# ddemidov/vexcl

Hardware: AMD Instinct MI355X
Metric: fp64 CSR SpMV GFLOP/s, 3D Poisson 512^3 (y = A*x through vex::SpMat's library object vexhip_spmat) (higher is better)
Workload: dtype f64

## Files before the change

### vexcl_amd/csrc/common.hpp

```cpp
#pragma once
#include <hip/hip_runtime.h>
#include <algorithm>
#include <chrono>
#include <cstdint>
#include <cstdio>
#include <cstdlib>
#include <string>

#include "../../include/vexhip.h"

namespace vexhip {

std::string &last_error();
int &last_error_code();
int fail(const char *file, int line, const std::string &what);

inline int check(hipError_t e, const char *file, int line) {
    if (e == hipSuccess) return 0;
    (void)hipGetLastError();
    const int rc = fail(file, line, std::string(hipGetErrorName(e)) + ": " + hipGetErrorString(e));
    last_error_code() = (int)e;
    return rc;
}

constexpr int kWave = 64;

inline hipStream_t as_stream(void *s) { return reinterpret_cast<hipStream_t>(s); }

struct device_info {
    int cus = 0;
    bool ok = false;
};
const device_info &info(int dev);


enum env_id {
    ENV_VEXCL_CACHE_DIR,
    ENV_VEXCL_CACHE_KERNELS,
    ENV_VEXCL_SHOW_KERNELS,
    ENV_VEXCL_SHOW_SCRATCH,
    ENV_VEXHIP_COMM_PEER,
    ENV_VEXHIP_DEBUG,
    ENV_VEXHIP_DIST_PACK,
    ENV_VEXHIP_FFT_EXTRA_LDS,
    ENV_VEXHIP_FFT_LANES_DIV,
    ENV_VEXHIP_FFT_NO_SINGLE,
    ENV_VEXHIP_FFT_ROW_ELEMS,
    ENV_VEXHIP_FFT_STRIDED_ELEMS,
    ENV_VEXHIP_GRID32_DEPTH,
    ENV_VEXHIP_GRID_2D_LINE,
    ENV_VEXHIP_GRID_BUILD_WGS,
    ENV_VEXHIP_GRID_SEGMENT,
    ENV_VEXHIP_HALO_ACQUIRE,
    ENV_VEXHIP_HALO_DEBUG,
    ENV_VEXHIP_HALO_DEPTH,
    ENV_VEXHIP_HALO_EDGE_PLANES,
    ENV_VEXHIP_HALO_HI_PLANES,
    ENV_VEXHIP_HALO_LO_PLANES,
    ENV_VEXHIP_HALO_NO_GHOST,
    ENV_VEXHIP_HALO_NO_PUSH,
    ENV_VEXHIP_HALO_PUSH_BLOCKS,
    ENV_VEXHIP_HALO_TWO_LAUNCHES,
    ENV_VEXHIP_HALO_TWO_PASS,
    ENV_VEXHIP_IPC_PUSH_PER_BLOCK,
    ENV_VEXHIP_IPC_TIMEOUT_MS,
    ENV_VEXHIP_IPC_WINDOW_MEM,
    ENV_VEXHIP_MALLOC_STAGGER,
    ENV_VEXHIP_MARCH_LDS,
    ENV_VEXHIP_MARCH_RUN,
    ENV_VEXHIP_NO_GRID,
    ENV_VEXHIP_NO_GRID_BUILD,
    ENV_VEXHIP_NO_PLANE512,
    ENV_VEXHIP_PLANE32_DEPTH,
    ENV_VEXHIP_PLANE_DEPTH,
    ENV_VEXHIP_PLANE_FORCE,
    ENV_VEXHIP_PLANE_STORE,
    ENV_VEXHIP_PLANE_TILE,
    ENV_VEXHIP_RCCL_SELF,
    ENV_VEXHIP_SELL_XLOAD,
    ENV_VEXHIP_SETUP_TRACE,
    ENV_COUNT
};
const char *env(env_id id);
void reload_env();

struct setup_trace {
    bool on; hipStream_t s; std::chrono::steady_clock::time_point t0, last;
    explicit setup_trace(hipStream_t st) : on(env(ENV_VEXHIP_SETUP_TRACE) != nullptr), s(st) { t0 = last = std::chrono::steady_clock::now(); }
    void mark(const char *what) {
        if (!on) return;
        (void)hipStreamSynchronize(s);
        const auto now = std::chrono::steady_clock::now();
        std::fprintf(stderr, "[vexhip set-up] %-28s %8.3f ms  (at %8.3f)\n", what,
                     std::chrono::duration<double, std::milli>(now - last).count(), std::chrono::duration<double, std::milli>(now - t0).count());
        last = now;
    }
};

template <typename T> struct dev_buf {
    T *p = nullptr;
    dev_buf() = default;
    dev_buf(const dev_buf &) = delete;
    dev_buf &operator=(const dev_buf &) = delete;
    ~dev_buf() { if (p) (void)hipFree(p); }
    hipError_t alloc(size_t count) { return hipMalloc(reinterpret_cast<void **>(&p), std::max<size_t>(count, 1) * sizeof(T)); }
    hipError_t free_now() { T *q = p; p = nullptr; return q ? hipFree(q) : hipSuccess; }
    T *release() { T *r = p; p = nullptr; return r; }
};

int scan_exclusive_i32_internal(int dev, hipStream_t s, const int *in, int *out, int64_t n);
int scan_exclusive_u32_tmp(hipStream_t s, const unsigned *in, unsigned *out, int64_t n, unsigned *tmp);
size_t scan_tmp_elems_u32(int64_t n);

}

#define VEXHIP_TRY(expr)                                                      \
    do {                                                                      \
        if (int _rc = ::vexhip::check((expr), __FILE__, __LINE__)) return _rc;\
    } while (0)

#define VEXHIP_REQUIRE(cond, msg)                                             \
    do {                                                                      \
        if (!(cond)) return ::vexhip::fail(__FILE__, __LINE__, msg);          \
    } while (0)

#define VEXHIP_SET_DEVICE(dev) VEXHIP_TRY(hipSetDevice(dev))

#define VEXHIP_WARM_TU(name)                                                   \
    namespace vexhip {                                                         \
    namespace { __global__ void warm_##name##_kernel() {} }                    \
    void warm_##name() { warm_##name##_kernel<<<1, 64>>>(); }                  \
    }

#define VEXHIP_LAUNCH_CHECK() VEXHIP_TRY(hipGetLastError())
```

### vexcl_amd/csrc/plane.hip

```cpp
#include "common.hpp"
#include "walk.hpp"
#include "halo.hpp"
#include "plane.hpp"
#include "storage.hpp"

#include <algorithm>
#include <cstdlib>
#include <cstring>
#include <vector>

namespace vexhip {
namespace {

constexpr int PL_LINE_B = PL_ROWS * 8;

__device__ __forceinline__ void push_piece(const double *__restrict__ x, int far, const halo_dev &H, unsigned long long step, bool down, int j,
        int per, unsigned target, bool counted, int *s_flag)
{
    const int t = threadIdx.x;
    if (t == 0) *s_flag = spin_until(down ? H.sent_lo : H.sent_hi, step - 1ull, H.err, H.ticks, 0) ? 1 : 0;
    __syncthreads();
    if (!*s_flag) return;
    const double *src = x + (down ? (long long)H.z0 * far : (long long)(H.z1 - 1) * far);
    double *dst = down ? H.dst_lo : H.dst_hi;
    const int i0 = j * per, i1 = i0 + per < H.halo ? i0 + per : H.halo;
    for (int i = i0 + 2 * t; i < i1; i += 512)
        *reinterpret_cast<d2 *>(dst + i) = *reinterpret_cast<const d2 *>(src + i);
    __builtin_amdgcn_fence(__ATOMIC_RELEASE, "workgroup");
    asm volatile("s_waitcnt vmcnt(0)" ::: "memory");
    __syncthreads();
    if (t == 0 && counted) {
        unsigned *cnt = H.done + (down ? 1 : 2);
        const unsigned old = __hip_atomic_fetch_add(cnt, 1u, __ATOMIC_RELAXED, __HIP_MEMORY_SCOPE_AGENT);
        if (old + 1u == target) {
            __hip_atomic_store(cnt, 0u, __ATOMIC_RELAXED, __HIP_MEMORY_SCOPE_AGENT);
            if (H.release) __builtin_amdgcn_fence(__ATOMIC_RELEASE, "");
            __hip_atomic_store(down ? H.peer_arrive_lo : H.peer_arrive_hi, step, __ATOMIC_RELAXED, __HIP_MEMORY_SCOPE_SYSTEM);
        }
    }
}

template <int TY, int ZM, int STORE_AUX, bool HALO, bool FLAT = false>
__device__ __forceinline__
void plane_walk(const double *__restrict__ x, double *__restrict__ y, double alpha, const double *__restrict__ zs, double beta,
        const int *__restrict__ blocks, const char *__restrict__ pool, const int *__restrict__ deltas, const double *__restrict__ values,
        const plane_dev &pd, const halo_dev &H, [[maybe_unused]] const unsigned long long step_in)
{
    __shared__ int s_slot[256];
    __shared__ double s_value[256];
    __shared__ double s_other[15][256];

    const int t = threadIdx.x;
    unsigned b = blockIdx.x;
    [[maybe_unused]] unsigned long long step = 0;
    [[maybe_unused]] __shared__ int s_flag[2];
    [[maybe_unused]] unsigned long long dbg_t0 = 0, dbg_flag = 0, dbg_data = 0;
    if constexpr (HALO) {
        if (H.debug) dbg_t0 = wall_clock64();
        step = step_in;
        halo_announce(H, step);
        const unsigned npush = H.pull ? 0u : (H.dst_lo ? (unsigned)H.push_blocks : 0u) + (H.dst_hi ? (unsigned)H.push_blocks : 0u);
        if (b < npush) {
            const bool down = H.dst_lo && b < (unsigned)H.push_blocks;
            const unsigned j = down ? b : b - (H.dst_lo ? (unsigned)H.push_blocks : 0u);
            const int per = ((H.halo + H.push_blocks - 1) / H.push_blocks + 511) / 512 * 512;
            push_piece(x, pd.far, H, step, down, (int)j, per, (unsigned)H.push_blocks, true, &s_flag[0]);
            if (H.debug && t == 0) { unsigned long long *d = H.debug + 6ull * blockIdx.x; d[0] = dbg_t0; d[1] = 0; d[2] = 0; d[3] = wall_clock64(); d[4] = ~0ull; d[5] = down ? 0ull : 1ull; }
            return;
        }
        b -= npush;
    }
    const unsigned xcd = b & 7u, q = b >> 3;
    const int zc = (int)(q / (unsigned)pd.tpx), tyl = (int)(q - (unsigned)zc * (unsigned)pd.tpx);
    const int tile = (int)xcd * pd.tpx + tyl;
    if (tile >= pd.tiles) return;
    const int y0 = TY * tile;
    int z, zend;
    [[maybe_unused]] bool second = false;
    [[maybe_unused]] int z2 = 0, zend2 = 0;
    if constexpr (HALO) {
        const int mid0 = H.z0 + H.lo_planes, mid1 = H.z1 - H.hi_planes;
        const int nmain = (mid1 - mid0 + pd.depth - 1) / pd.depth;
        if (zc < nmain) { z = mid0 + zc * pd.depth; zend = z + pd.depth < mid1 ? z + pd.depth : mid1; }
        else if (H.hi_planes && zc == nmain) { z = mid1; zend = H.z1; }
        else if (H.lo_two_pass && mid0 - H.z0 >= 2) {
            z = H.z0 + 1; zend = mid0; second = true; z2 = H.z0; zend2 = H.z0 + 1;
        } else { z = H.z0; zend = mid0; }
    } else {
        z = zc * pd.depth;
        zend = z + pd.depth < pd.nz ? z + pd.depth : pd.nz;
    }
    if (z >= zend) return;
    [[maybe_unused]] const int z_first0 = z, mid_end = zend;
    if constexpr (HALO) {
        if (!H.pull && H.push_blocks == 0 && b < 512u) {
            const bool down = b < 256u;
            double *dst = down ? H.dst_lo : H.dst_hi;
            if (dst) {
                const int per = ((H.halo + 255) / 256 + 511) / 512 * 512, j = (int)(b & 255u);
                push_piece(x, pd.far, H, step, down, j, per, (unsigned)((H.halo + per - 1) / per), j * per < H.halo, &s_flag[0]);
                __syncthreads();
            }
        }
    }
    const int ny = pd.ny;
    const int nslices = (int)pd.nslices, xlines = (int)pd.xlines;
    const long long x_last = pd.x_last;
    const unsigned lane_b = 16u * (unsigned)t;
    const int edge_b = (t >> 6) * 1024 + ((t & 63) == 63 ? 1024 : -8);

    s_slot[t] = 2 * position_of(deltas[t], pd.far); s_value[t] = values[t];
    __syncthreads();

    const int wp = (pd.w + 1) >> 1;
    auto decode = [&](int blk) -> unsigned {
        if (pd.pitch > 0) return decode_table<false>(pool + (long long)blk * 7 * pd.pitch + 2 * t, pd.pitch, s_value, s_other, t);
        const unsigned *cw = reinterpret_cast<const unsigned *>(pool + (long long)blk * ((long long)wp * 2048)) + t;
        unsigned dcw[4], vcw[4];
#pragma unroll
        for (int u = 0; u < 4; ++u) { dcw[u] = u < wp ? cw[u * 256] : 0xffffffffu; vcw[u] = u < wp ? cw[(wp + u) * 256] : 0u; }
#pragma unroll
        for (int p = 0; p < 14; ++p) s_other[p][t] = 0.0;
        unsigned bits = 0;
#pragma unroll
        for (int j = 0; j < 8; ++j) {
            const unsigned cword = dcw[j >> 1] >> (16 * (j & 1)), vword = vcw[j >> 1] >> (16 * (j & 1));
#pragma unroll
            for (int r = 0; r < 2; ++r) {
                const unsigned code = j < pd.w ? (cword >> (8 * r)) & 255u : 255u;
                const bool real = code < PL_PAD_FIRST;
                const int slot = real ? s_slot[code] + r : 14;
                s_other[slot][t] = s_value[real ? (vword >> (8 * r)) & 255u : 255u];
                bits |= (real ? 1u : 0u) << slot;
            }
        }
        return bits & 0x3fffu;
    };

    const int hot = pd.hot;
    double aH[7][2];
    unsigned long long mH[7][2];
    take_hot(decode(hot), s_other, t, aH, mH);
    unsigned bitsO = 0;
    int other = -1;

    const int line_lo = HALO ? H.z0 * ny : 0, line_hi = HALO ? H.z1 * ny : xlines;
    const int yline_hi = HALO ? H.z1 * ny : nslices;
    [[maybe_unused]] bool got_lo = false, got_hi = false, ghost_bad = false;
    auto line_of = [&](int zz, int l) -> int {
        int li = zz * ny + (y0 - 1 + l);
        li = li < line_lo ? line_lo : li; li = li >= line_hi ? line_hi - 1 : li;
        return li;
    };
    auto ld = [&](int zz, int l) -> d2 {
        if constexpr (HALO) {
            const int li = zz * ny + (y0 - 1 + l);
            if (li < line_lo || li >= line_hi) {
                const bool below = li < line_lo;
                const int gl = below ? li - (line_lo - ny) : li - line_hi;
                const double *g = below ? H.lo : H.hi;
                d2 r = {0.0, 0.0};
                if (!g || gl < 0 || gl >= ny || l == 0 || l == TY + 1) return r;
                bool &got = below ? got_lo : got_hi;
                if (!got && H.pull != 2) {
                    if (t == 0) s_flag[below ? 0 : 1] = spin_until(below ? H.arrive_lo : H.arrive_hi, step, H.err, H.ticks, H.acquire) ? 1 : 0;
                    __syncthreads();
                    if (!s_flag[below ? 0 : 1]) ghost_bad = true;
                    got = true;
                    if (H.debug && !dbg_flag) dbg_flag = wall_clock64();
                }
                if (ghost_bad) { r.x = r.y = __builtin_nan(""); return r; }
                if (H.debug && !dbg_data) {
                    const d2 v = *reinterpret_cast<const d2 *>(reinterpret_cast<const char *>(g + (long long)gl * PL_ROWS) + lane_b);
                    asm volatile("s_waitcnt vmcnt(0)" :: "v"(v.x), "v"(v.y) : "memory");
                    dbg_data = wall_clock64();
                    return v;
                }
                return *reinterpret_cast<const d2 *>(reinterpret_cast<const char *>(g + (long long)gl * PL_ROWS) + lane_b);
            }
        }
        const char *p = reinterpret_cast<const char *>(x + (long long)line_of(zz, l) * PL_ROWS);
        return *reinterpret_cast<const d2 *>(p + lane_b);
    };
    auto edge = [&](int zz, int l) -> double {
        if constexpr (HALO) {
            const int li = zz * ny + (y0 - 1 + l);
            if (li < line_lo || li >= line_hi) return 0.0;
            long long i = (long long)li * PL_ROWS + (edge_b >> 3);
            const long long a = (long long)line_lo * PL_ROWS, e = (long long)line_hi * PL_ROWS - 1;
            i = i < a ? a : i; i = i > e ? e : i;
            return x[i];
        }
        long long i = (long long)line_of(zz, l) * PL_ROWS + (edge_b >> 3);
        i = i < 0 ? 0 : i; i = i > x_last ? x_last : i;
        return x[i];
    };
    auto yold = [&](int zz, int l) -> d2 {
        int li = zz * ny + (y0 + l);
        li = li < line_lo ? line_lo : li; li = li >= yline_hi ? yline_hi - 1 : li;
        return *reinterpret_cast<const d2 *>(reinterpret_cast<const char *>(zs + (long long)li * PL_ROWS) + lane_b);
    };

    constexpr int NPASS = HALO ? 2 : 1;
    for (int pass = 0; pass < NPASS; ++pass) {
    if constexpr (HALO) if (pass == 1) { if (!second) break; z = z2; zend = zend2; }
    d2 Cs[4][TY], Hs[2][2], Yo[TY];
    double Es[2][TY];
    const unsigned plane_b32 = (unsigned)ny * (unsigned)PL_LINE_B;
    const int z_first = z;
    const __amdgpu_buffer_rsrc_t rx = __builtin_amdgcn_make_buffer_rsrc(
        const_cast<double *>(x + ((long long)z_first * ny + (y0 - 1)) * PL_ROWS), 0, -1, 0x00020000);
    const __amdgpu_buffer_rsrc_t ry = __builtin_amdgcn_make_buffer_rsrc(y + ((long long)z_first * ny + y0) * PL_ROWS, 0, -1, 0x00020000);
    [[maybe_unused]] const __amdgpu_buffer_rsrc_t rz = __builtin_amdgcn_make_buffer_rsrc(const_cast<double *>(ZM == 1 ? zs : x) + ((long long)z_first * ny + y0) * PL_ROWS, 0, -1, 0x00020000);
    fill_registers<ZM>(Cs, Hs, Es, Yo, z, !FLAT, ld, edge, yold);

    int zh = zend;
    {
        const int a = (line_hi - 1 - TY - y0) / ny - 3, bb = (yline_hi - TY - y0) / ny - (ZM == 1 ? 1 : 0);
        if (line_hi - 1 - TY - y0 < 0 || yline_hi - TY - y0 < 0) zh = 0;
        else { zh = zh < a + 1 ? zh : a + 1; zh = zh < bb + 1 ? zh : bb + 1; }
    }

    while (z < zend) {
        unsigned long long use_hot[TY];
        const int run = fast_run(blocks, ny, y0, TY, z, zh, hot, other, t, use_hot);
        if (run >= 4) {
            unsigned xo = (unsigned)((z + 2 - z_first) * plane_b32), yo = (unsigned)((z - z_first) * plane_b32);
            auto fast_step = [&](d2 (&P)[TY], d2 (&C)[TY], d2 (&N)[TY], d2 (&Hl)[2], double (&E)[TY]) {
                d2 o[TY];
#pragma unroll
                for (int l = 0; l < TY; ++l) {
                    double xs[2][7], s[2] = {};
                    stencil_x(P, C, N, Hl, E, l, xs);
                    if (use_hot[l] & 1ull) hot_sums(s, aH, mH, xs); else other_sums(s, s_other, t, bitsO, xs);
                    o[l] = add_addend<ZM>(alpha, s, beta, Yo[l], C[l]);
                }
#pragma unroll
                for (int l = 0; l < TY; ++l) use_hot[l] >>= 1;
#pragma unroll
                for (int l = 0; l < TY; ++l) store16<STORE_AUX>(o[l], ry, (int)lane_b, yo + l * PL_LINE_B);
                if (ZM == 1) {
#pragma unroll
                    for (int l = 0; l < TY; ++l) Yo[l] = load16<double>(rz, (int)lane_b, yo + plane_b32 + l * PL_LINE_B);
                }
                if constexpr (!FLAT) {
                    Hl[0] = load16<double>(rx, (int)lane_b, xo);
                    Hl[1] = load16<double>(rx, (int)lane_b, xo + (TY + 1) * PL_LINE_B);
                }
#pragma unroll
                for (int l = 0; l < TY; ++l) {
                    P[l] = load16<double>(rx, (int)lane_b, xo + plane_b32 + (l + 1) * PL_LINE_B);
                    E[l] = load_edge<double>(rx, edge_b + 8, xo + (l + 1) * PL_LINE_B - 8u);
                }
                xo += plane_b32; yo += plane_b32; ++z;
            };
            for (int g = run >> 2; g > 0; --g) fast_group(fast_step, Cs, Hs, Es);
            if (run == 64) continue;
        }
        if (z >= zend) break;
#pragma unroll
        for (int l = 0; l < TY; ++l) {
            const int li = z * ny + (y0 + l);
            if (li < yline_hi) {
                double xs[2][7], s[2] = {};
                stencil_x(Cs[0], Cs[1], Cs[2], Hs[0], Es[0], l, xs);
                const int blk = __builtin_amdgcn_readfirstlane(blocks[li]);
                if (blk == hot) hot_sums(s, aH, mH, xs);
                else {
                    if (blk != other) { bitsO = decode(blk); other = blk; }
                    other_sums(s, s_other, t, bitsO, xs);
                }
                const d2 o = add_addend<ZM>(alpha, s, beta, Yo[l], Cs[1][l]);
                __builtin_nontemporal_store(o, reinterpret_cast<d2 *>(reinterpret_cast<char *>(y + (long long)li * PL_ROWS) + lane_b));
            }
        }
        rotate_by_copy<ZM>(Cs, Hs, Es, Yo, z, !FLAT, ld, edge, yold);
        ++z;
    }
    }
    if constexpr (HALO) {
        if (H.debug && t == 0) {
            unsigned long long *d = H.debug + 6ull * blockIdx.x;
            d[0] = dbg_t0; d[1] = dbg_flag; d[2] = dbg_data; d[3] = wall_clock64(); d[4] = (unsigned long long)(second ? z2 : z_first0); d[5] = (unsigned long long)(second ? mid_end : zend);
        }
    }
}

#ifndef VEXHIP_HALO_WAVES
#define VEXHIP_HALO_WAVES 2
#endif
template <int TY, int ZM, int STORE_AUX, bool HALO = false, bool FLAT = false>
__global__ __launch_bounds__(256, (TY == 2 && !HALO) ? 4 : (HALO ? VEXHIP_HALO_WAVES : 2))
void sell8_plane_kernel(const double *__restrict__ x, double *__restrict__ y, double alpha, const double *__restrict__ zs, double beta,
        const int *__restrict__ blocks, const char *__restrict__ pool, const int *__restrict__ deltas, const double *__restrict__ values,
        plane_dev pd, halo_dev H)
{
    if constexpr (!HALO) {
        plane_walk<TY, ZM, STORE_AUX, false, FLAT>(x, y, alpha, zs, beta, blocks, pool, deltas, values, pd, H, 0ull);
    } else {
        const unsigned long long step = *H.step;
        plane_walk<TY, ZM, STORE_AUX, true>(x, y, alpha, zs, beta, blocks, pool, deltas, values, pd, H, step);
        halo_finish(H, step);
    }
}

__global__ __launch_bounds__(256)
void stream_copy_kernel(const double *__restrict__ x, double *__restrict__ y, long long npairs, long long n) {
    const long long i = (long long)blockIdx.x * 256 + threadIdx.x;
    if (i < npairs) __builtin_nontemporal_store(reinterpret_cast<const d2 *>(x)[i], reinterpret_cast<d2 *>(y) + i);
    else if (i == npairs && (n & 1)) y[n - 1] = x[n - 1];
}

__global__ void halo_signal_kernel(halo_dev H) {
    const unsigned long long step = *H.step;
    if (H.consumed_lo) __hip_atomic_store(H.consumed_lo, step, __ATOMIC_RELEASE, __HIP_MEMORY_SCOPE_SYSTEM);
    if (H.consumed_hi) __hip_atomic_store(H.consumed_hi, step, __ATOMIC_RELEASE, __HIP_MEMORY_SCOPE_SYSTEM);
    if (H.pull == 1) {
        if (H.sent_lo) (void)spin_until(H.sent_lo, step, H.err, H.ticks, 0);
        if (H.sent_hi) (void)spin_until(H.sent_hi, step, H.err, H.ticks, 0);
    }
    *H.step = step + 1ull;
}

}
}

namespace vexhip {
int plane_apply_axpby(int dev, void *stream, int64_t n, double alpha, int zm, const double *zs, double beta, int64_t w, const void *pool,
        const int32_t *blocks, const int32_t *deltas, const double *values, const double *x, double *y, const vexhip_plane *plane)
{
    if (int rc = plane_check(plane, 0, PL_LINE_B, n, w, pool && blocks && deltas && values, x, y, true)) return rc;
    VEXHIP_REQUIRE(zm == 0 || zm == 2 || (zm == 1 && zs && (reinterpret_cast<uintptr_t>(zs) & 15) == 0), "plane product: the addend must be a 16-byte aligned vector");
    VEXHIP_SET_DEVICE(dev);
    const plane_dev pd = plane_launch(*plane, n, w, plane->tile, plane->depth);
    unsigned grid;
    if (int rc = plane_workgroups(pd, pd.nz, 0, 0, &grid)) return rc;
    const char *cpool = static_cast<const char *>(pool);
    with_launch_forms(zm, plane->store_policy, [&](auto ZM, auto AUX) {
        auto kernel = plane->tile == 4 ? sell8_plane_kernel<4, ZM(), AUX()> : plane->flat ? sell8_plane_kernel<2, ZM(), AUX(), false, true> : sell8_plane_kernel<2, ZM(), AUX()>;
        kernel<<<grid, 256, 0, as_stream(stream)>>>(x, y, alpha, zs, beta, blocks, cpool, deltas, values, pd, halo_dev());
    });
    VEXHIP_LAUNCH_CHECK();
    return 0;
}

}

using namespace vexhip;

static bool plane_geometry_with(long long cus, long long ny, long long nz, int hot, vexhip_plane *out);
static bool plane_geometry(int dev, long long ny, long long nz, int hot, vexhip_plane *out)
{
    return plane_geometry_with(std::max(1, info(dev).cus), ny, nz, hot, out);
}
static bool plane_geometry_with(long long cus, long long ny, long long nz, int hot, vexhip_plane *out)
{
    cus = std::max(1ll, cus);
    auto depth_for = [&](long long tl) {
        const long long tiles = ny / tl;
        long long chunks = std::max(1ll, std::min(nz / 8, (cus + tiles / 2) / tiles));
        if (tiles * chunks > cus || tiles * chunks * 20 < cus * 19) {
            double best = 0;
            const long long cmax = std::max(1ll, nz / 16);
            for (long long c = 1; c <= cmax; ++c) {
                const long long per_cu = (tiles * c + cus - 1) / cus;
                if (per_cu < 6 && c < cmax) continue;
                const double est = (double)per_cu * (double)((nz + c - 1) / c + 6);
                if (best == 0 || est <= best * 1.01) { if (best == 0 || est < best) best = est; chunks = c; }
                if (per_cu > 24) break;
            }
        }
        if (chunks == 1 && nz >= 32 && nz <= 192 && tiles * 2 <= 2 * cus) chunks = 2;
        return (nz + chunks - 1) / chunks;
    };
    long long tile = 2;
    if (const char *e = env(ENV_VEXHIP_PLANE_TILE)) tile = (std::atoi(e) == 4 && ny % 4 == 0) ? 4 : 2;
    long long depth = depth_for(tile);
    if (const char *e = env(ENV_VEXHIP_PLANE_DEPTH)) depth = std::max(1, std::atoi(e));
    depth = std::min(depth, nz);
    while ((depth + 4) * ny * PL_LINE_B >= (1ll << 32) && depth > 8) depth = (depth + 1) / 2;
    if ((depth + 4) * ny * PL_LINE_B >= (1ll << 32)) return false;
    out->lines_per_plane = (int32_t)ny; out->planes = (int32_t)nz; out->depth = (int32_t)depth; out->hot_block = hot; out->tile = (int32_t)tile;
    out->store_policy = tile == 4 ? 2 : 1;
    if (const char *e = env(ENV_VEXHIP_PLANE_STORE)) out->store_policy = std::max(0, std::min(3, std::atoi(e)));
    return true;
}

namespace vexhip {
int plane_plan_from_grid(int dev, const vexhip_grid *grid, int64_t rows, vexhip_plane *out)
{
    VEXHIP_REQUIRE(grid && out, "NULL argument");
    std::memset(out, 0, sizeof(*out));
    const bool force = env(ENV_VEXHIP_PLANE_FORCE) != nullptr;
    if (!grid->usable || grid->nx != PL_ROWS || grid->segments != 1 || rows % PL_ROWS != 0) return 0;
    const long long ny = grid->lines_per_plane, nz = grid->planes;
    if (ny < 4 || ny % 2 != 0 || (nz < 4 && !force) || (rows / PL_ROWS < 64 && !force)) return 0;
    if ((grid->x_last + 1) % PL_ROWS != 0 || grid->x_last + 1 < rows) return 0;
    if (!plane_geometry(dev, ny, nz, grid->hot_class, out)) return 0;
    out->table_pitch = grid->pitch;
    out->flat = grid->flat;
    out->x_last = grid->x_last; out->usable = 1;
    return 0;
}
}

namespace vexhip {
int plane_apply_halo(int dev, hipStream_t s, int64_t n_ext, double alpha, int append, int64_t w, const void *pool, const int32_t *blocks,
        const int32_t *deltas, const double *values, const double *x, double *y, const vexhip_plane *plane, halo_dev H)
{
    if (int rc = plane_check(plane, 2, PL_LINE_B, n_ext, w, pool && blocks && deltas && values, x, y, true)) return rc;
    if (int rc = check_halo_step(H, plane->planes, (long long)plane->lines_per_plane * PL_ROWS, false)) return rc;
    VEXHIP_SET_DEVICE(dev);
    const int nzr = H.z1 - H.z0;
    int edge_planes = 8;
    if (const char *e = env(ENV_VEXHIP_HALO_EDGE_PLANES)) edge_planes = std::max(1, std::atoi(e));
    int lo_planes = edge_planes, hi_planes = edge_planes;
    if (const char *e = env(ENV_VEXHIP_HALO_LO_PLANES)) lo_planes = std::max(1, std::atoi(e));
    if (const char *e = env(ENV_VEXHIP_HALO_HI_PLANES)) hi_planes = std::max(1, std::atoi(e));
    H.lo_planes = H.lo ? std::min(lo_planes, nzr) : 0;
    H.hi_planes = H.hi ? std::min(hi_planes, nzr - H.lo_planes) : 0;
    const int mid = nzr - H.lo_planes - H.hi_planes;
    int depth = std::max(1, mid);
    if (const char *e = env(ENV_VEXHIP_HALO_DEPTH)) depth = std::max(1, std::atoi(e));
    const plane_dev pd = plane_launch(*plane, n_ext, w, 2, depth);
    const long long npush = H.pull ? 0 : (H.dst_lo ? H.push_blocks : 0) + (H.dst_hi ? H.push_blocks : 0);
    unsigned grid;
    if (int rc = plane_workgroups(pd, mid, (H.lo_planes ? 1 : 0) + (H.hi_planes ? 1 : 0), npush, &grid)) return rc;
    VEXHIP_REQUIRE(H.pull || H.push_blocks > 0 || grid - npush >= 512 || !(H.dst_lo || H.dst_hi), "too few workgroups to push the boundary planes");
    const double *xe = x - (long long)H.z0 * pd.far;
    double *ye = y - (long long)H.z0 * pd.far;
    const char *cpool = static_cast<const char *>(pool);
    auto kernel = append ? sell8_plane_kernel<2, 1, 18, true> : sell8_plane_kernel<2, 0, 18, true>;
    kernel<<<grid, 256, 0, s>>>(xe, ye, alpha, append ? ye : nullptr, append ? 1.0 : 0.0, blocks, cpool, deltas, values, pd, H);
    VEXHIP_LAUNCH_CHECK();
    if (H.pull != 2 && !H.one_launch) {
        halo_signal_kernel<<<1, 1, 0, s>>>(H);
        VEXHIP_LAUNCH_CHECK();
    }
    return 0;
}
}

extern "C" {

int vexhip_sell8_plane_geometry(int cus, int64_t lines_per_plane, int64_t planes, vexhip_plane *out)
{
    VEXHIP_REQUIRE(out, "NULL output");
    std::memset(out, 0, sizeof(*out));
    reload_env();
    VEXHIP_REQUIRE(lines_per_plane >= 4 && lines_per_plane % 2 == 0 && lines_per_plane < (1ll << 30) && planes >= 1 && planes < (1ll << 30), "bad grid");
    if (!plane_geometry_with(cus, lines_per_plane, planes, 0, out)) { std::memset(out, 0, sizeof(*out)); return 0; }
    return 0;
}

int vexhip_sell8_plane_plan(int dev, void *stream, const int32_t *deltas, int ndeltas, const int32_t *blocks, int64_t nslices,
        const void *pool, int64_t dictionary_blocks, int64_t ell_width, int64_t rows, int64_t tail_nnz, int value_bytes,
        int64_t x_last, vexhip_plane *out)
{
    VEXHIP_REQUIRE(out, "NULL output");
    std::memset(out, 0, sizeof(*out));
    reload_env();
    const bool force = env(ENV_VEXHIP_PLANE_FORCE) != nullptr;
    if ((value_bytes != 8 && value_bytes != 4) || !deltas || !blocks || !pool || ndeltas < 2 || ndeltas > 7 || dictionary_blocks < 1 || dictionary_blocks > 128) return 0;
    if (ell_width < 1 || ell_width > 8 || tail_nnz != 0 || rows != nslices * PL_ROWS || (nslices < 64 && !force)) return 0;
    if (x_last < 0 || (x_last + 1) % PL_ROWS != 0 || x_last + 1 < rows) return 0;
    VEXHIP_SET_DEVICE(dev);
    hipStream_t s = as_stream(stream);
    const int wp = (int)((ell_width + 1) / 2);
    const size_t code_bytes = (size_t)wp * 2048;
    std::vector<int> table((size_t)ndeltas), id((size_t)nslices);
    std::vector<unsigned> codes((size_t)dictionary_blocks * code_bytes / 4);
    VEXHIP_TRY(hipMemcpyAsync(table.data(), deltas, sizeof(int) * (size_t)ndeltas, hipMemcpyDeviceToHost, s));
    VEXHIP_TRY(hipMemcpyAsync(id.data(), blocks, sizeof(int) * (size_t)nslices, hipMemcpyDeviceToHost, s));
    VEXHIP_TRY(hipMemcpyAsync(codes.data(), pool, (size_t)dictionary_blocks * code_bytes, hipMemcpyDeviceToHost, s));
    VEXHIP_TRY(hipStreamSynchronize(s));
    long long far = 0;
    for (int d : table) {
        const long long a = std::llabs((long long)d);
        if (a == 0 || a == 1 || a == PL_ROWS) continue;
        if (far == 0) far = a;
        if (a != far) return 0;
    }
    if (far < 4 * PL_ROWS || far % (2 * PL_ROWS) != 0 || far > (1ll << 30)) return 0;
    const long long ny = far / PL_ROWS, nz = (nslices + ny - 1) / ny;
    if (nz < 4 && !force) return 0;
    auto position = [&](int d) { return d == 0 ? 3 : d == -1 ? 2 : d == 1 ? 4 : d == -PL_ROWS ? 1 : d == PL_ROWS ? 5 : d == -far ? 0 : 6; };
    for (int64_t blk = 0; blk < dictionary_blocks; ++blk) {
        const unsigned *cw = codes.data() + (size_t)blk * code_bytes / 4;
        for (int t = 0; t < 256; ++t)
            for (int r = 0; r < 2; ++r) {
                int last = -1;
                for (int j = 0; j < (int)ell_width; ++j) {
                    const unsigned cword = cw[(size_t)(j >> 1) * 256 + t] >> (16 * (j & 1));
                    const unsigned code = (cword >> (8 * r)) & 255u;
                    if (code >= PL_PAD_FIRST) continue;
                    if ((int)code >= ndeltas) return 0;
                    const int p = position(table[code]);
                    if (p <= last) return 0;
                    last = p;
                }
            }
    }
    std::vector<int64_t> uses((size_t)dictionary_blocks, 0);
    for (int64_t k = 0; k < nslices; ++k) {
        if (id[(size_t)k] < 0 || id[(size_t)k] >= dictionary_blocks) return 0;
        ++uses[(size_t)id[(size_t)k]];
    }
    const int hot = (int)(std::max_element(uses.begin(), uses.end()) - uses.begin());
    if ((nslices - uses[(size_t)hot]) * 16 > nslices && !force) return 0;
    if (!plane_geometry(dev, ny, nz, hot, out)) return 0;
    out->flat = 1;
    for (int d : table) if (std::llabs((long long)d) == PL_ROWS) out->flat = 0;
    out->x_last = x_last; out->usable = 1;
    return 0;
}

int vexhip_spmv_sell8v_plane_f64_i32(int dev, void *stream, int64_t n, double alpha, int append, int64_t w, const void *pool,
        const int32_t *blocks, const int32_t *deltas, const double *values, const double *x, double *y, const vexhip_plane *plane)
{ return plane_apply<double>(dev, stream, n, alpha, append, w, pool, blocks, deltas, values, x, y, plane); }

int vexhip_stream_copy_f64(int dev, void *stream, const double *x, double *y, int64_t n)
{
    VEXHIP_REQUIRE(n >= 0 && (n == 0 || (x && y)), "bad copy arguments");
    VEXHIP_REQUIRE((reinterpret_cast<uintptr_t>(x) & 15) == 0 && (reinterpret_cast<uintptr_t>(y) & 15) == 0, "stream copy: x and y must be 16-byte aligned");
    if (n == 0) return 0;
    VEXHIP_SET_DEVICE(dev);
    const long long npairs = n / 2, grid = (npairs + 1 + 255) / 256;
    VEXHIP_REQUIRE(grid < (1ll << 31), "vector too large for one launch");
    stream_copy_kernel<<<(unsigned)grid, 256, 0, as_stream(stream)>>>(x, y, npairs, (long long)n);
    VEXHIP_LAUNCH_CHECK();
    return 0;
}

}

VEXHIP_WARM_TU(plane)
```

### vexcl_amd/csrc/runtime.hip

```cpp
#include "common.hpp"

#include <hip/hiprtc.h>

#include <atomic>
#include <cerrno>
#include <cstdlib>
#include <cstring>
#include <fstream>
#include <mutex>
#include <sstream>
#include <unordered_map>
#include <vector>
#include <sys/stat.h>
#include <unistd.h>

namespace vexhip {

std::string &last_error() {
    static thread_local std::string s;
    return s;
}

int &last_error_code() {
    static thread_local int c = 0;
    return c;
}

int fail(const char *file, int line, const std::string &what) {
    std::ostringstream o;
    o << file << ":" << line << "\n\t" << what;
    last_error() = o.str();
    last_error_code() = 0;
    return 1;
}

void warm_misc();
void warm_reduce();
void warm_scan();
void warm_sort();
void warm_stencil();
void warm_ccsr();
void warm_sell8();
void warm_plane();
void warm_plane32();
void warm_grid();
void warm_grid32();
void warm_spmm();
void warm_spmv();
void warm_split();
void warm_comm();
void warm_fft();
void warm_mba();

const device_info &info(int dev) {
    static std::mutex mx;
    static device_info cache[64];
    static device_info fallback;
    std::lock_guard<std::mutex> lock(mx);
    if (dev < 0 || dev >= 64) { fallback.cus = 256; return fallback; }
    if (!cache[dev].ok) {
        hipDeviceProp_t p;
        if (hipGetDeviceProperties(&p, dev) == hipSuccess) {
            cache[dev].cus = p.multiProcessorCount;
            cache[dev].ok = true;
            hipStreamCaptureMode cmode = hipStreamCaptureModeRelaxed;
            const bool swapped = hipThreadExchangeStreamCaptureMode(&cmode) == hipSuccess;
            int cur = -1;
            if (hipGetDevice(&cur) == hipSuccess && hipSetDevice(dev) == hipSuccess) {
                void *d = nullptr;
                if (hipMalloc(&d, 1 << 16) == hipSuccess) {
                    std::vector<char> h(1 << 16);
                    (void)hipMemcpy(h.data(), d, h.size(), hipMemcpyDeviceToHost);
                    (void)hipMemcpy(d, h.data(), h.size(), hipMemcpyHostToDevice);
                    (void)hipFree(d);
                }
                warm_misc(); warm_reduce(); warm_scan(); warm_sort(); warm_stencil(); warm_ccsr(); warm_sell8(); warm_plane(); warm_plane32(); warm_grid(); warm_grid32(); warm_spmm(); warm_spmv(); warm_split(); warm_comm(); warm_fft(); warm_mba();
                (void)hipDeviceSynchronize();
                (void)hipGetLastError();
                (void)hipSetDevice(cur);
            }
            if (swapped) (void)hipThreadExchangeStreamCaptureMode(&cmode);
        } else {
            cache[dev].cus = 256;
        }
    }
    return cache[dev];
}

}

using namespace vexhip;

namespace {

std::atomic<uint64_t> g_compiled{0}, g_disk_hits{0};

std::string digest(const std::string &s) {
    uint64_t h1 = 0xcbf29ce484222325ull, h2 = 0x84222325cbf29ce4ull;
    for (unsigned char c : s) {
        h1 = (h1 ^ c) * 0x100000001b3ull;
        h2 = (h2 ^ (c + 0x9e)) * 0x100000001b3ull;
        h2 ^= h2 >> 29;
    }
    char buf[40];
    std::snprintf(buf, sizeof(buf), "%016llx%016llx", (unsigned long long)h1, (unsigned long long)h2);
    return buf;
}

std::string cache_root() {
    if (const char *e = env(ENV_VEXCL_CACHE_DIR)) return e;
    const char *home = std::getenv("HOME");
    return std::string(home ? home : "/tmp") + "/.vexcl_amd";
}

bool cache_enabled() {
    const char *e = env(ENV_VEXCL_CACHE_KERNELS);
    return !(e && e[0] == '0');
}

bool mkdirs(const std::string &path) {
    std::string cur;
    for (size_t i = 0; i < path.size(); ++i) {
        cur += path[i];
        if (path[i] == '/' || i + 1 == path.size())
            if (::mkdir(cur.c_str(), 0755) != 0 && errno != EEXIST) return false;
    }
    return true;
}

bool read_file(const std::string &p, std::vector<char> &out) {
    std::ifstream f(p, std::ios::binary);
    if (!f) return false;
    f.seekg(0, std::ios::end);
    std::streamsize n = f.tellg();
    if (n <= 0) return false;
    f.seekg(0);
    out.resize((size_t)n);
    return (bool)f.read(out.data(), n);
}

void write_file_atomic(const std::string &dir, const std::string &name, const std::vector<char> &data) {
    if (!mkdirs(dir)) return;
    std::string tmp = dir + "/." + name + "." + std::to_string((long)::getpid());
    {
        std::ofstream f(tmp, std::ios::binary);
        if (!f) return;
        f.write(data.data(), (std::streamsize)data.size());
        if (!f) { ::unlink(tmp.c_str()); return; }
    }
    if (::rename(tmp.c_str(), (dir + "/" + name).c_str()) != 0) ::unlink(tmp.c_str());
}

int rtc_fail(const char *file, int line, hiprtcResult r, const std::string &log) {
    return fail(file, line, std::string("hiprtc: ") + hiprtcGetErrorString(r) + (log.empty() ? "" : "\n" + log));
}

}

namespace vexhip {
namespace {
const char *const kEnvNames[ENV_COUNT] = {
    "VEXCL_CACHE_DIR",
    "VEXCL_CACHE_KERNELS",
    "VEXCL_SHOW_KERNELS",
    "VEXCL_SHOW_SCRATCH",
    "VEXHIP_COMM_PEER",
    "VEXHIP_DEBUG",
    "VEXHIP_DIST_PACK",
    "VEXHIP_FFT_EXTRA_LDS",
    "VEXHIP_FFT_LANES_DIV",
    "VEXHIP_FFT_NO_SINGLE",
    "VEXHIP_FFT_ROW_ELEMS",
    "VEXHIP_FFT_STRIDED_ELEMS",
    "VEXHIP_GRID32_DEPTH",
    "VEXHIP_GRID_2D_LINE",
    "VEXHIP_GRID_BUILD_WGS",
    "VEXHIP_GRID_SEGMENT",
    "VEXHIP_HALO_ACQUIRE",
    "VEXHIP_HALO_DEBUG",
    "VEXHIP_HALO_DEPTH",
    "VEXHIP_HALO_EDGE_PLANES",
    "VEXHIP_HALO_HI_PLANES",
    "VEXHIP_HALO_LO_PLANES",
    "VEXHIP_HALO_NO_GHOST",
    "VEXHIP_HALO_NO_PUSH",
    "VEXHIP_HALO_PUSH_BLOCKS",
    "VEXHIP_HALO_TWO_LAUNCHES",
    "VEXHIP_HALO_TWO_PASS",
    "VEXHIP_IPC_PUSH_PER_BLOCK",
    "VEXHIP_IPC_TIMEOUT_MS",
    "VEXHIP_IPC_WINDOW_MEM",
    "VEXHIP_MALLOC_STAGGER",
    "VEXHIP_MARCH_LDS",
    "VEXHIP_MARCH_RUN",
    "VEXHIP_NO_GRID",
    "VEXHIP_NO_GRID_BUILD",
    "VEXHIP_NO_PLANE512",
    "VEXHIP_PLANE32_DEPTH",
    "VEXHIP_PLANE_DEPTH",
    "VEXHIP_PLANE_FORCE",
    "VEXHIP_PLANE_STORE",
    "VEXHIP_PLANE_TILE",
    "VEXHIP_RCCL_SELF",
    "VEXHIP_SELL_XLOAD",
    "VEXHIP_SETUP_TRACE",
};
struct env_snapshot { bool set[ENV_COUNT]; char text[ENV_COUNT][96]; };
env_snapshot g_env;
std::mutex g_env_mx;
std::once_flag g_env_once;
void read_env() {
    std::lock_guard<std::mutex> lock(g_env_mx);
    for (int i = 0; i < ENV_COUNT; ++i) {
        const char *v = std::getenv(kEnvNames[i]);
        const bool set = v != nullptr;
        if (set == g_env.set[i] && (!set || std::strncmp(g_env.text[i], v, sizeof(g_env.text[i]) - 1) == 0)) continue;
        if (set) { std::strncpy(g_env.text[i], v, sizeof(g_env.text[i]) - 1); g_env.text[i][sizeof(g_env.text[i]) - 1] = 0; }
        g_env.set[i] = set;
    }
}
}
const char *env(env_id id) {
    std::call_once(g_env_once, read_env);
    return g_env.set[id] ? g_env.text[id] : nullptr;
}
void reload_env() {
    std::call_once(g_env_once, read_env);
    read_env();
}
}


extern "C" {

const char *vexhip_last_error(void) { return last_error().c_str(); }
int vexhip_last_error_code(void) { return last_error_code(); }
int vexhip_abi_version(void) { return VEXHIP_ABI_VERSION; }

int vexhip_device_count(int *count) {
    VEXHIP_REQUIRE(count, "count is NULL");
    hipError_t e = hipGetDeviceCount(count);
    if (e == hipErrorNoDevice) { *count = 0; (void)hipGetLastError(); return 0; }
    VEXHIP_TRY(e);
    return 0;
}

int vexhip_device_get_props(int dev, vexhip_device_props *out) {
    VEXHIP_REQUIRE(out, "props is NULL");
    hipDeviceProp_t p;
    VEXHIP_TRY(hipGetDeviceProperties(&p, dev));
    std::memset(out, 0, sizeof(*out));
    std::strncpy(out->name, p.name, sizeof(out->name) - 1);
    std::strncpy(out->arch, p.gcnArchName, sizeof(out->arch) - 1);
    out->compute_units = p.multiProcessorCount;
    out->wavefront_size = p.warpSize;
    out->max_threads_per_block = p.maxThreadsPerBlock;
    out->lds_bytes_per_block = (int32_t)p.sharedMemPerBlock;
    out->clock_khz = p.clockRate;
    out->l2_bytes = p.l2CacheSize;
    out->global_mem_bytes = p.totalGlobalMem;
    out->pci_bus_id = p.pciBusID;
    return 0;
}

int vexhip_device_sync(int dev) {
    VEXHIP_SET_DEVICE(dev);
    VEXHIP_TRY(hipDeviceSynchronize());
    return 0;
}

int vexhip_mem_info(int dev, uint64_t *free_bytes, uint64_t *total_bytes) {
    VEXHIP_SET_DEVICE(dev);
    size_t f = 0, t = 0;
    VEXHIP_TRY(hipMemGetInfo(&f, &t));
    if (free_bytes) *free_bytes = f;
    if (total_bytes) *total_bytes = t;
    return 0;
}

int vexhip_stream_create(int dev, void **stream) {
    VEXHIP_REQUIRE(stream, "stream is NULL");
    VEXHIP_SET_DEVICE(dev);
    hipStream_t s;
    VEXHIP_TRY(hipStreamCreateWithFlags(&s, hipStreamNonBlocking));
    *stream = s;
    return 0;
}

int vexhip_stream_destroy(int dev, void *stream) {
    VEXHIP_SET_DEVICE(dev);
    VEXHIP_TRY(hipStreamDestroy(as_stream(stream)));
    return 0;
}

int vexhip_stream_sync(int dev, void *stream) {
    VEXHIP_SET_DEVICE(dev);
    VEXHIP_TRY(hipStreamSynchronize(as_stream(stream)));
    return 0;
}

int vexhip_event_create(int dev, int timing, void **event) {
    VEXHIP_REQUIRE(event, "event is NULL");
    VEXHIP_SET_DEVICE(dev);
    hipEvent_t e;
    VEXHIP_TRY(hipEventCreateWithFlags(&e, timing ? hipEventDefault : hipEventDisableTiming));
    *event = e;
    return 0;
}

int vexhip_event_destroy(int dev, void *event) {
    VEXHIP_SET_DEVICE(dev);
    VEXHIP_TRY(hipEventDestroy((hipEvent_t)event));
    return 0;
}

int vexhip_event_record(int dev, void *event, void *stream) {
    VEXHIP_SET_DEVICE(dev);
    VEXHIP_TRY(hipEventRecord((hipEvent_t)event, as_stream(stream)));
    return 0;
}

int vexhip_event_sync(int dev, void *event) {
    VEXHIP_SET_DEVICE(dev);
    VEXHIP_TRY(hipEventSynchronize((hipEvent_t)event));
    return 0;
}

int vexhip_stream_wait_event(int dev, void *stream, void *event) {
    VEXHIP_SET_DEVICE(dev);
    VEXHIP_TRY(hipStreamWaitEvent(as_stream(stream), (hipEvent_t)event, 0));
    return 0;
}

int vexhip_event_elapsed_ms(int dev, void *start, void *stop, float *ms) {
    VEXHIP_SET_DEVICE(dev);
    VEXHIP_TRY(hipEventElapsedTime(ms, (hipEvent_t)start, (hipEvent_t)stop));
    return 0;
}


static constexpr size_t kStaggerAlign = size_t(64) << 20, kStaggerStep = size_t(2) << 20, kStaggerSlots = 5, kStaggerFrom = size_t(64) << 20;

extern "C" size_t vexhip_malloc_stagger(size_t bytes, unsigned ordinal) {
    if (bytes < kStaggerFrom) return 0;
    static const bool off = env(ENV_VEXHIP_MALLOC_STAGGER) && std::atoi(env(ENV_VEXHIP_MALLOC_STAGGER)) == 0;
    if (off) return 0;
    return (ordinal % kStaggerSlots) * kStaggerStep;
}
extern "C" size_t vexhip_malloc_placement(size_t bytes, uint64_t raw_address, unsigned ordinal) {
    if (bytes < kStaggerFrom) return 0;
    const uint64_t aligned = (raw_address + kStaggerAlign - 1) / kStaggerAlign * kStaggerAlign;
    return (size_t)(aligned - raw_address) + vexhip_malloc_stagger(bytes, ordinal);
}

namespace {
std::mutex g_alloc_mx;
std::unordered_map<void *, void *> g_alloc_base;
std::atomic<unsigned> g_alloc_ordinal{0};
}

int vexhip_reload_env(void) { reload_env(); return 0; }

int vexhip_malloc(int dev, size_t bytes, void **ptr) {
    VEXHIP_REQUIRE(ptr, "ptr is NULL");
    VEXHIP_SET_DEVICE(dev);
    *ptr = nullptr;
    if (bytes == 0) return 0;
    static const bool off = env(ENV_VEXHIP_MALLOC_STAGGER) && std::atoi(env(ENV_VEXHIP_MALLOC_STAGGER)) == 0;
    if (bytes < kStaggerFrom || off) { VEXHIP_TRY(hipMalloc(ptr, bytes)); return 0; }
    void *raw = nullptr;
    VEXHIP_TRY(hipMalloc(&raw, bytes + kStaggerAlign + (kStaggerSlots - 1) * kStaggerStep));
    const size_t shift = vexhip_malloc_placement(bytes, (uint64_t)reinterpret_cast<uintptr_t>(raw), g_alloc_ordinal.fetch_add(1));
    void *p = static_cast<char *>(raw) + shift;
    if (p != raw) { std::lock_guard<std::mutex> lock(g_alloc_mx); g_alloc_base[p] = raw; }
    *ptr = p;
    return 0;
}

int vexhip_malloc_managed(int dev, size_t bytes, void **ptr) {
    VEXHIP_REQUIRE(ptr, "ptr is NULL");
    VEXHIP_SET_DEVICE(dev);
    *ptr = nullptr;
    if (bytes == 0) return 0;
    VEXHIP_TRY(hipMallocManaged(ptr, bytes, hipMemAttachGlobal));
    return 0;
}

int vexhip_free(int dev, void *ptr) {
    if (!ptr) return 0;
    VEXHIP_SET_DEVICE(dev);
    {
        std::lock_guard<std::mutex> lock(g_alloc_mx);
        auto it = g_alloc_base.find(ptr);
        if (it != g_alloc_base.end()) { ptr = it->second; g_alloc_base.erase(it); }
    }
    VEXHIP_TRY(hipFree(ptr));
    return 0;
}

int vexhip_memcpy_h2d(int dev, void *dst, const void *src, size_t bytes, void *stream, int blocking) {
    if (!bytes) return 0;
    VEXHIP_SET_DEVICE(dev);
    VEXHIP_TRY(hipMemcpyAsync(dst, src, bytes, hipMemcpyHostToDevice, as_stream(stream)));
    if (blocking) VEXHIP_TRY(hipStreamSynchronize(as_stream(stream)));
    return 0;
}

int vexhip_memcpy_d2h(int dev, void *dst, const void *src, size_t bytes, void *stream, int blocking) {
    if (!bytes) return 0;
    VEXHIP_SET_DEVICE(dev);
    VEXHIP_TRY(hipMemcpyAsync(dst, src, bytes, hipMemcpyDeviceToHost, as_stream(stream)));
    if (blocking) VEXHIP_TRY(hipStreamSynchronize(as_stream(stream)));
    return 0;
}

int vexhip_memcpy_d2d(int dev, void *dst, const void *src, size_t bytes, void *stream) {
    if (!bytes) return 0;
    VEXHIP_SET_DEVICE(dev);
    VEXHIP_TRY(hipMemcpyAsync(dst, src, bytes, hipMemcpyDeviceToDevice, as_stream(stream)));
    return 0;
}

int vexhip_memcpy_peer(int dst_dev, void *dst, int src_dev, const void *src, size_t bytes, void *stream) {
    if (!bytes) return 0;
    VEXHIP_SET_DEVICE(dst_dev);
    if (dst_dev == src_dev)
        VEXHIP_TRY(hipMemcpyAsync(dst, src, bytes, hipMemcpyDeviceToDevice, as_stream(stream)));
    else
        VEXHIP_TRY(hipMemcpyPeerAsync(dst, dst_dev, src, src_dev, bytes, as_stream(stream)));
    return 0;
}

int vexhip_memset(int dev, void *ptr, int byte, size_t bytes, void *stream) {
    if (!bytes) return 0;
    VEXHIP_SET_DEVICE(dev);
    VEXHIP_TRY(hipMemsetAsync(ptr, byte, bytes, as_stream(stream)));
    return 0;
}

int vexhip_host_alloc(size_t bytes, void **ptr) {
    VEXHIP_REQUIRE(ptr, "ptr is NULL");
    VEXHIP_TRY(hipHostMalloc(ptr, bytes ? bytes : 1, hipHostMallocDefault));
    return 0;
}

int vexhip_host_free(void *ptr) {
    if (!ptr) return 0;
    VEXHIP_TRY(hipHostFree(ptr));
    return 0;
}


int vexhip_module_compile(int dev, const char *source, const char *options, void **module) {
    reload_env();
    VEXHIP_REQUIRE(source && module, "source/module is NULL");
    VEXHIP_SET_DEVICE(dev);
    hipDeviceProp_t prop;
    VEXHIP_TRY(hipGetDeviceProperties(&prop, dev));
    std::string arch = prop.gcnArchName;
    std::string opts = options ? options : "";

    if (const char *show = env(ENV_VEXCL_SHOW_KERNELS))
        if (show[0] != '0') std::printf("%s\n", source);

    int rtc_major = 0, rtc_minor = 0;
    hiprtcVersion(&rtc_major, &rtc_minor);
    std::string key = digest(std::string(source) + "\x01" + opts + "\x01" + arch + "\x01" +
                             std::to_string(rtc_major) + "." + std::to_string(rtc_minor));
    std::string dir = cache_root() + "/" + key.substr(0, 2) + "/" + key.substr(2);

    std::vector<char> code;
    bool from_disk = cache_enabled() && read_file(dir + "/kernel.hsaco", code);

    if (!from_disk) {
        hiprtcProgram prog;
        hiprtcResult r = hiprtcCreateProgram(&prog, source, "vexcl_kernel.hip", 0, nullptr, nullptr);
        if (r != HIPRTC_SUCCESS) return rtc_fail(__FILE__, __LINE__, r, "");

        std::vector<std::string> ostr;
        ostr.push_back("--offload-arch=" + arch);
        ostr.push_back("-O3");
        ostr.push_back("-std=c++17");
        {
            std::istringstream is(opts);
            std::string tok;
            while (is >> tok) ostr.push_back(tok);
        }
        std::vector<const char *> oc;
        for (auto &s : ostr) oc.push_back(s.c_str());

        r = hiprtcCompileProgram(prog, (int)oc.size(), oc.data());
        if (r != HIPRTC_SUCCESS) {
            size_t ls = 0;
            hiprtcGetProgramLogSize(prog, &ls);
            std::string log(ls, '\0');
            if (ls) hiprtcGetProgramLog(prog, &log[0]);
            hiprtcDestroyProgram(&prog);
            std::fprintf(stderr, "%s\n%s\n", source, log.c_str());
            return rtc_fail(__FILE__, __LINE__, r, log);
        }
        size_t cs = 0;
        r = hiprtcGetCodeSize(prog, &cs);
        if (r != HIPRTC_SUCCESS) { hiprtcDestroyProgram(&prog); return rtc_fail(__FILE__, __LINE__, r, ""); }
        code.resize(cs);
        r = hiprtcGetCode(prog, code.data());
// ... 99 lines not shown
```

Baseline: 4716.

## Add look-ahead plane walk kernel with four-deep block-class prefetch for TY=2

```diff
diff --git a/vexcl_amd/csrc/common.hpp b/vexcl_amd/csrc/common.hpp
--- a/vexcl_amd/csrc/common.hpp
+++ b/vexcl_amd/csrc/common.hpp
@@ -76,6 +76,7 @@
     ENV_VEXHIP_PLANE_FORCE,
     ENV_VEXHIP_PLANE_STORE,
     ENV_VEXHIP_PLANE_TILE,
+    ENV_VEXHIP_PLANE_WALK,
     ENV_VEXHIP_RCCL_SELF,
     ENV_VEXHIP_SELL_XLOAD,
     ENV_VEXHIP_SETUP_TRACE,
diff --git a/vexcl_amd/csrc/plane.hip b/vexcl_amd/csrc/plane.hip
--- a/vexcl_amd/csrc/plane.hip
+++ b/vexcl_amd/csrc/plane.hip
@@ -304,6 +304,204 @@
     }
 }
 
+template <int ZM, int STORE_AUX>
+__device__ __forceinline__
+void plane_walk_ahead(const double *__restrict__ x, double *__restrict__ y, double alpha, const double *__restrict__ zs, double beta,
+        const int *__restrict__ blocks, const char *__restrict__ pool, const int *__restrict__ deltas, const double *__restrict__ values,
+        const plane_dev &pd)
+{
+    constexpr int TY = 2;
+    __shared__ int s_slot[256];
+    __shared__ double s_value[256];
+    __shared__ double s_other[15][256];
+
+    const int t = threadIdx.x;
+    const unsigned b = blockIdx.x;
+    const unsigned xcd = b & 7u, q = b >> 3;
+    const int zc = (int)(q / (unsigned)pd.tpx), tyl = (int)(q - (unsigned)zc * (unsigned)pd.tpx);
+    const int tile = (int)xcd * pd.tpx + tyl;
+    if (tile >= pd.tiles) return;
+    const int y0 = TY * tile;
+    int z = zc * pd.depth;
+    const int zend = z + pd.depth < pd.nz ? z + pd.depth : pd.nz;
+    if (z >= zend) return;
+    const int ny = pd.ny;
+    const int nslices = (int)pd.nslices, xlines = (int)pd.xlines;
+    const long long x_last = pd.x_last;
+    const unsigned lane_b = 16u * (unsigned)t;
+    const int edge_b = (t >> 6) * 1024 + ((t & 63) == 63 ? 1024 : -8);
+
+    auto line_of = [&](int zz, int l) -> int {
+        int li = zz * ny + (y0 - 1 + l);
+        li = li < 0 ? 0 : li; li = li >= xlines ? xlines - 1 : li;
+        return li;
+    };
+    auto ld = [&](int zz, int l) -> d2 {
+        return *reinterpret_cast<const d2 *>(reinterpret_cast<const char *>(x + (long long)line_of(zz, l) * PL_ROWS) + lane_b);
+    };
+    auto edge = [&](int zz, int l) -> double {
+        long long i = (long long)line_of(zz, l) * PL_ROWS + (edge_b >> 3);
+        i = i < 0 ? 0 : i; i = i > x_last ? x_last : i;
+        return x[i];
+    };
+    auto yold = [&](int zz, int l) -> d2 {
+        int li = zz * ny + (y0 + l);
+        li = li < 0 ? 0 : li; li = li >= nslices ? nslices - 1 : li;
+        return *reinterpret_cast<const d2 *>(reinterpret_cast<const char *>(zs + (long long)li * PL_ROWS) + lane_b);
+    };
+
+    d2 Cs[4][TY], Hs[2][2], Yo[TY];
+    double Es[2][TY];
+    const unsigned plane_b32 = (unsigned)ny * (unsigned)PL_LINE_B;
+    const int z_first = z;
+    const __amdgpu_buffer_rsrc_t rx = __builtin_amdgcn_make_buffer_rsrc(
+        const_cast<double *>(x + ((long long)z_first * ny + (y0 - 1)) * PL_ROWS), 0, -1, 0x00020000);
+    const __amdgpu_buffer_rsrc_t ry = __builtin_amdgcn_make_buffer_rsrc(y + ((long long)z_first * ny + y0) * PL_ROWS, 0, -1, 0x00020000);
+    [[maybe_unused]] const __amdgpu_buffer_rsrc_t rz = __builtin_amdgcn_make_buffer_rsrc(const_cast<double *>(ZM == 1 ? zs : x) + ((long long)z_first * ny + y0) * PL_ROWS, 0, -1, 0x00020000);
+    int zh = zend;
+    {
+        const int a = (xlines - 1 - TY - y0) / ny - 3, bb = (nslices - TY - y0) / ny - (ZM == 1 ? 1 : 0);
+        if (xlines - 1 - TY - y0 < 0 || nslices - TY - y0 < 0) zh = 0;
+        else { zh = zh < a + 1 ? zh : a + 1; zh = zh < bb + 1 ? zh : bb + 1; }
+    }
+
+    fill_registers<ZM>(Cs, Hs, Es, Yo, z, true, ld, edge, yold);
+    int cw[4][TY];
+    auto class_of = [&](int zz, int l) -> int {
+        const int li = zz * ny + (y0 + l);
+        return __builtin_amdgcn_readfirstlane(blocks[li < nslices ? li : nslices - 1]);
+    };
+#pragma unroll
+    for (int i = 0; i < 4; ++i)
+#pragma unroll
+        for (int l = 0; l < TY; ++l) cw[i][l] = class_of(z + i, l);
+
+    s_slot[t] = 2 * position_of(deltas[t], pd.far); s_value[t] = values[t];
+    __syncthreads();
+    const int wp = (pd.w + 1) >> 1;
+    auto decode = [&](int blk) -> unsigned {
+        if (pd.pitch > 0) return decode_table<false>(pool + (long long)blk * 7 * pd.pitch + 2 * t, pd.pitch, s_value, s_other, t);
+        const unsigned *cw = reinterpret_cast<const unsigned *>(pool + (long long)blk * ((long long)wp * 2048)) + t;
+        unsigned dcw[4], vcw[4];
+#pragma unroll
+        for (int u = 0; u < 4; ++u) { dcw[u] = u < wp ? cw[u * 256] : 0xffffffffu; vcw[u] = u < wp ? cw[(wp + u) * 256] : 0u; }
+#pragma unroll
+        for (int p = 0; p < 14; ++p) s_other[p][t] = 0.0;
+        unsigned bits = 0;
+#pragma unroll
+        for (int j = 0; j < 8; ++j) {
+            const unsigned cword = dcw[j >> 1] >> (16 * (j & 1)), vword = vcw[j >> 1] >> (16 * (j & 1));
+#pragma unroll
+            for (int r = 0; r < 2; ++r) {
+                const unsigned code = j < pd.w ? (cword >> (8 * r)) & 255u : 255u;
+                const bool real = code < PL_PAD_FIRST;
+                const int slot = real ? s_slot[code] + r : 14;
+                s_other[slot][t] = s_value[real ? (vword >> (8 * r)) & 255u : 255u];
+                bits |= (real ? 1u : 0u) << slot;
+            }
+        }
+        return bits & 0x3fffu;
+    };
+    const int hot = pd.hot;
+    double aH[7][2];
+    unsigned long long mH[7][2];
+    take_hot(decode(hot), s_other, t, aH, mH);
+    unsigned bitsO = 0;
+    int other = -1;
+#pragma unroll
+    for (int l = TY - 1; l >= 0; --l)
+        if (cw[0][l] != hot && z * ny + (y0 + l) < nslices) other = cw[0][l];
+    if (other >= 0) bitsO = decode(other);
+
+    unsigned use_hot = 0;
+    auto look = [&]() -> bool {
+        bool fast = z + 4 <= zh;
+        use_hot = 0;
+#pragma unroll
+        for (int l = 0; l < TY; ++l)
+#pragma unroll
+            for (int i = 0; i < 4; ++i) {
+                fast = fast && (cw[i][l] == hot || cw[i][l] == other);
+                use_hot |= (cw[i][l] == hot ? 1u : 0u) << (4 * l + i);
+            }
+        return fast;
+    };
+    while (z < zend) {
+        if (look()) {
+            __builtin_amdgcn_s_waitcnt(0x0f70);
+            do {
+#pragma unroll
+                for (int i = 0; i < 4; ++i)
+#pragma unroll
+                    for (int l = 0; l < TY; ++l) cw[i][l] = class_of(z + 4 + i, l);
+                unsigned xo = (unsigned)((z + 2 - z_first) * plane_b32), yo = (unsigned)((z - z_first) * plane_b32);
+                auto fast_step = [&](d2 (&P)[TY], d2 (&C)[TY], d2 (&N)[TY], d2 (&Hl)[2], double (&E)[TY]) {
+                    d2 o[TY];
+#pragma unroll
+                    for (int l = 0; l < TY; ++l) {
+                        double xs[2][7], sm[2] = {};
+                        stencil_x(P, C, N, Hl, E, l, xs);
+                        if (use_hot & (1u << (4 * l))) hot_sums(sm, aH, mH, xs); else other_sums(sm, s_other, t, bitsO, xs);
+                        o[l] = add_addend<ZM>(alpha, sm, beta, Yo[l], C[l]);
+                    }
+                    use_hot >>= 1;
+#pragma unroll
+                    for (int l = 0; l < TY; ++l) store16<STORE_AUX>(o[l], ry, (int)lane_b, yo + l * PL_LINE_B);
+                    if (ZM == 1) {
+#pragma unroll
+                        for (int l = 0; l < TY; ++l) Yo[l] = load16<double>(rz, (int)lane_b, yo + plane_b32 + l * PL_LINE_B);
+                    }
+                    Hl[0] = load16<double>(rx, (int)lane_b, xo);
+                    Hl[1] = load16<double>(rx, (int)lane_b, xo + (TY + 1) * PL_LINE_B);
+#pragma unroll
+                    for (int l = 0; l < TY; ++l) {
+                        P[l] = load16<double>(rx, (int)lane_b, xo + plane_b32 + (l + 1) * PL_LINE_B);
+                        E[l] = load_edge<double>(rx, edge_b + 8, xo + (l + 1) * PL_LINE_B - 8u);
+                    }
+                    xo += plane_b32; yo += plane_b32; ++z;
+                };
+                fast_group(fast_step, Cs, Hs, Es);
+            } while (look());
+            if (z >= zend) break;
+        }
+#pragma unroll
+        for (int l = 0; l < TY; ++l) {
+            const int li = z * ny + (y0 + l);
+            if (li < nslices) {
+                double xs[2][7], sm[2] = {};
+                stencil_x(Cs[0], Cs[1], Cs[2], Hs[0], Es[0], l, xs);
+                const int blk = cw[0][l];
+                if (blk == hot) hot_sums(sm, aH, mH, xs);
+                else {
+                    if (blk != other) { bitsO = decode(blk); other = blk; }
+                    other_sums(sm, s_other, t, bitsO, xs);
+                }
+                const d2 o = add_addend<ZM>(alpha, sm, beta, Yo[l], Cs[1][l]);
+                __builtin_nontemporal_store(o, reinterpret_cast<d2 *>(reinterpret_cast<char *>(y + (long long)li * PL_ROWS) + lane_b));
+            }
+        }
+        rotate_by_copy<ZM>(Cs, Hs, Es, Yo, z, true, ld, edge, yold);
+        ++z;
+#pragma unroll
+        for (int l = 0; l < TY; ++l) {
+#pragma unroll
+            for (int i = 0; i < 3; ++i) cw[i][l] = cw[i + 1][l];
+            cw[3][l] = class_of(z + 3, l);
+        }
+    }
+}
+
+namespace ahead {
+template <int ZM, int STORE_AUX>
+__global__ __launch_bounds__(256, 4)
+void sell8_plane_kernel(const double *__restrict__ x, double *__restrict__ y, double alpha, const double *__restrict__ zs, double beta,
+        const int *__restrict__ blocks, const char *__restrict__ pool, const int *__restrict__ deltas, const double *__restrict__ values,
+        plane_dev pd)
+{
+    plane_walk_ahead<ZM, STORE_AUX>(x, y, alpha, zs, beta, blocks, pool, deltas, values, pd);
+}
+}
+
 __global__ __launch_bounds__(256)
 void stream_copy_kernel(const double *__restrict__ x, double *__restrict__ y, long long npairs, long long n) {
     const long long i = (long long)blockIdx.x * 256 + threadIdx.x;
@@ -336,7 +534,13 @@
     unsigned grid;
     if (int rc = plane_workgroups(pd, pd.nz, 0, 0, &grid)) return rc;
     const char *cpool = static_cast<const char *>(pool);
+    const char *walk = env(ENV_VEXHIP_PLANE_WALK);
+    const bool ahead = plane->tile == 2 && !plane->flat && !(walk && std::atoi(walk) == 0);
     with_launch_forms(zm, plane->store_policy, [&](auto ZM, auto AUX) {
+        if (ahead) {
+            ahead::sell8_plane_kernel<ZM(), AUX()><<<grid, 256, 0, as_stream(stream)>>>(x, y, alpha, zs, beta, blocks, cpool, deltas, values, pd);
+            return;
+        }
         auto kernel = plane->tile == 4 ? sell8_plane_kernel<4, ZM(), AUX()> : plane->flat ? sell8_plane_kernel<2, ZM(), AUX(), false, true> : sell8_plane_kernel<2, ZM(), AUX()>;
         kernel<<<grid, 256, 0, as_stream(stream)>>>(x, y, alpha, zs, beta, blocks, cpool, deltas, values, pd, halo_dev());
     });
diff --git a/vexcl_amd/csrc/runtime.hip b/vexcl_amd/csrc/runtime.hip
--- a/vexcl_amd/csrc/runtime.hip
+++ b/vexcl_amd/csrc/runtime.hip
@@ -201,6 +201,7 @@
     "VEXHIP_PLANE_FORCE",
     "VEXHIP_PLANE_STORE",
     "VEXHIP_PLANE_TILE",
+    "VEXHIP_PLANE_WALK",
     "VEXHIP_RCCL_SELF",
     "VEXHIP_SELL_XLOAD",
     "VEXHIP_SETUP_TRACE",
```

New measurement: 4961, median of 6. +5.2%, better.
